# Nazukixv/LiteASR

Measured on AMD Instinct MI355X. Metric: utterances/sec (U2-Conformer+CTC, 80-d fbank T≈1000) at 1/2/4/8 MI355X, higher is better.
Workload: dtype bf16; 1 GPU; U2-Conformer-small hybrid CTC-attention training step (fwd+loss+bwd+allreduce+clip+Noam/Adam); model=U2 enc 12x conformer d256 H4 ff2048, dec 6x, V 4233, global_batch=32, per_gpu_batch=32, seq_len=1000, label_len=40, parallelism=dp1, launch=hipgraph, ranks_seen=1, rank_launcher=env

## Files before the change

### liteasr_amd/csrc/gemm.hip

```cpp
#include "gemm_kernel.h"
#include <algorithm>


template <bool AKC, bool BKC, typename TC>
void launch_bf16(const GemmP& p, int BM, int BN, int ks, int nw, bool glds, dim3 grid, hipStream_t st);
#define LASR_EXTERN_LAUNCH(ak, bk)                                                                         \
  extern template void launch_bf16<ak, bk, float>(const GemmP&, int, int, int, int, bool, dim3, hipStream_t); \
  extern template void launch_bf16<ak, bk, bf16_t>(const GemmP&, int, int, int, int, bool, dim3, hipStream_t);
LASR_EXTERN_LAUNCH(true, true)
LASR_EXTERN_LAUNCH(true, false)
LASR_EXTERN_LAUNCH(false, true)
LASR_EXTERN_LAUNCH(false, false)
#undef LASR_EXTERN_LAUNCH

template <typename TC>
static void dispatch(const GemmP& p, bool akc, bool bkc, int bf16in, int BM, int BN, int ks, int nw, bool glds,
                     dim3 grid, hipStream_t st) {
  if (bf16in) {
    if (akc && bkc) launch_bf16<true, true, TC>(p, BM, BN, ks, nw, glds, grid, st);
    else if (akc) launch_bf16<true, false, TC>(p, BM, BN, ks, nw, glds, grid, st);
    else if (bkc) launch_bf16<false, true, TC>(p, BM, BN, ks, nw, glds, grid, st);
    else launch_bf16<false, false, TC>(p, BM, BN, ks, nw, glds, grid, st);
  } else {
    if (akc && bkc) gemm_f32_kernel<true, true, TC><<<grid, 256, 0, st>>>(p);
// ... 191 lines not shown
  LASR_CHECK_ARG(grid.y <= 65535 && grid.z <= 65535, "lasr_gemm: grid too large");
  const bool rs_fused = a->rowsum && glds && !akc;
  if (rs_fused) {
    p.rowsum = a->rowsum;
    if (split > 1) p.rs_ws = p.ws + (int64_t)split * batch * a->M * a->N;
  }
  if (a->c_dtype == LASR_F32) dispatch<float>(p, akc, bkc, bf, BM, BN, ks, nw, glds, grid, st);
  else dispatch<bf16_t>(p, akc, bkc, bf, BM, BN, ks, nw, glds, grid, st);
  int rc = lasr_check_launch("lasr_gemm");
  if (!rc && split > 1 && a->split_k >= 0 && post) {
    const int r = post->launch(p, post->ctx, st);
    if (r < 0) return r;
    post->done = r;
    if (r) {
      rc = lasr_check_launch("lasr_gemm/splitk_reduce_post");
      if (rc || !a->rowsum || rs_fused) return rc;
    }
  }
  if (!rc && split > 1 && a->split_k >= 0 && !(post && post->done)) {
    const int64_t total = (int64_t)a->M * a->N * batch;
    const int nblk = (int)std::min<int64_t>(cdiv(p.v4 ? total / 4 : total, 256), 4096);
    if (a->c_dtype == LASR_F32) splitk_reduce_kernel<float><<<nblk, 256, 0, st>>>(p);
    else splitk_reduce_kernel<bf16_t><<<nblk, 256, 0, st>>>(p);
    rc = lasr_check_launch("lasr_gemm/splitk_reduce");
  }
  if (rc || !a->rowsum || rs_fused) return rc;
  const int64_t used = split > 1 ? (int64_t)split * batch * a->M * a->N : 0;
  LASR_CHECK_ARG(a->workspace && a->workspace_bytes / 4 > used, "lasr_gemm: no workspace left for the rowsum");
  return lasr_colsum(a->A, a->in_dtype, a->K, a->M, a->lda_k, a->rowsum, 1, (float*)a->workspace + used,
                     a->workspace_bytes / 4 - used, stream);
}


int launch_dw_group(const DwGroupP& g, int BM, int BN, int blocks, hipStream_t st);
static int dw_group_lpt = 1;
extern "C" int lasr_gemm_dw_group_order(int longest_first) {
  dw_group_lpt = longest_first != 0;
  return LASR_OK;
}

extern "C" int lasr_gemm_dw_group(const lasr_gemm_args* args, int n, void* stream) {
  LASR_CHECK_ARG(args && n >= 1 && n <= LASR_DW_GROUP_MAX, "lasr_gemm_dw_group: 1..%d problems", LASR_DW_GROUP_MAX);
  DwGroupP g = {};
  g.n = n;
  int ord[LASR_DW_GROUP_MAX];
  int64_t work[LASR_DW_GROUP_MAX];
  for (int i = 0; i < n; ++i) {
    const lasr_gemm_args* a = args + i;
    int bm, bn, sp, ks;
    gemm_plan(a, &bm, &bn, &sp, &ks);
    work[i] = a->split_k == 1 || sp <= 1 ? a->K : cdiv(a->K, sp);
    ord[i] = i;
  }
  if (dw_group_lpt)
    std::stable_sort(ord, ord + n, [&](int x, int y) { return work[x] > work[y]; });
  int BM0 = 0, BN0 = 0, blocks = 0;
  for (int i = 0; i < n; ++i) {
    const lasr_gemm_args* a = args + ord[i];
    LASR_CHECK_ARG(a->in_dtype == LASR_BF16 && a->c_dtype == LASR_F32, "lasr_gemm_dw_group: bf16 in, fp32 partials");
    LASR_CHECK_ARG(a->lda_m == 1 && a->lda_k != 1 && a->ldb_n == 1 && a->ldb_k != 1,
                   "lasr_gemm_dw_group: A M-contiguous and B N-contiguous (dW = dY^T X)");
    const bool direct = a->split_k == 1;
    LASR_CHECK_ARG((direct || (a->split_k < 0 && a->workspace)) && (a->batch <= 1) && a->M > 0 && a->N > 0 &&
                       a->K > 0,
                   "lasr_gemm_dw_group: partials-only problems with a workspace, or direct (split_k 1) ones");
    LASR_CHECK_ARG(!direct || (a->C && a->ldc >= a->N && (a->beta == 0.f || a->beta == 1.f) && a->alpha == 1.f &&
                               !a->alpha_dev),
                   "lasr_gemm_dw_group: a direct problem needs C, ldc >= N, beta 0 or 1, alpha 1");
    LASR_CHECK_ARG(i == 0 || direct == (g.direct[0] != 0), "lasr_gemm_dw_group: direct and split problems mixed");
    LASR_CHECK_ARG(!a->act && !a->zout && !a->aux && !a->res && a->drop_p <= 0.f && !a->bias,
                   "lasr_gemm_dw_group: no epilogue");
    LASR_CHECK_ARG(gemm_uses_glds(a), "lasr_gemm_dw_group: operands not LDS-DMA eligible");
    int BM, BN, split, ks;
    gemm_plan(a, &BM, &BN, &split, &ks);
    if (direct) split = 2;
    LASR_CHECK_ARG(split > 1, "lasr_gemm_dw_group: plan is not a split-K launch");
    if (((BM == 128 && BN == 64) || (BM == 64 && BN == 128)) && a->M >= 128 && a->N >= 128) {
      BM = BN = 128;
      if (a->M >= 256 && a->N >= 256 && !direct) {
        BM = 256;
        BN = 128;
      }
    }
    LASR_CHECK_ARG(i == 0 || (BM == BM0 && BN == BN0), "lasr_gemm_dw_group: problems plan different tiles");
    BM0 = BM;
    BN0 = BN;
    if (direct) split = 1;
    g.M[i] = a->M; g.N[i] = a->N; g.K[i] = a->K;
    g.split[i] = split;
    g.kchunk[i] = direct ? a->K : (int)(cdiv(cdiv(a->K, split), 32) * 32);
    g.direct[i] = direct;
    g.C[i] = (float*)a->C; g.ldc[i] = a->ldc; g.beta[i] = a->beta; g.rowsum[i] = a->rowsum;
    g.v4[i] = a->N % 4 == 0 && aligned16(direct ? a->C : a->workspace);
    g.A[i] = a->A; g.lda[i] = a->lda_k;
    g.B[i] = a->B; g.ldb[i] = a->ldb_k;
    g.ws[i] = (float*)a->workspace;
    g.rs_ws[i] = a->rowsum && !direct ? (float*)a->workspace + (int64_t)split * a->M * a->N : nullptr;
    g.start[i] = blocks;
    const int64_t nb = cdiv(a->M, BM) * cdiv(a->N, BN) * (int64_t)split;
    LASR_CHECK_ARG(blocks + nb + 8 < (1ll << 31), "lasr_gemm_dw_group: too many blocks");
    blocks += (int)cdiv(nb, 8) * 8;
  }
  g.start[n] = blocks;
  static const int slice_xcd = [] { const char* e = getenv("LASR_DW_SLICE_XCD"); return e && e[0] ? atoi(e) : 1; }();
  g.slice_xcd = slice_xcd;
  LASR_CHECK_ARG(launch_dw_group(g, BM0, BN0, blocks, (hipStream_t)stream) == 0,
                 "lasr_gemm_dw_group: no grouped instance for tile %dx%d", BM0, BN0);
  return lasr_check_launch("lasr_gemm_dw_group");
}
```

### liteasr_amd/csrc/gemm_group.hip

```cpp
#include "gemm_kernel.h"

int launch_dw_group(const DwGroupP& g, int BM, int BN, int blocks, hipStream_t st) {
  if (BM == 64 && BN == 64) gemm_dw_group_kernel<64, 64, 3, 3><<<blocks, 256, 0, st>>>(g);
  else if (BM == 64 && BN == 128) gemm_dw_group_kernel<64, 128, 3, 2><<<blocks, 256, 0, st>>>(g);
  else if (BM == 128 && BN == 64) gemm_dw_group_kernel<128, 64, 3, 2><<<blocks, 256, 0, st>>>(g);
  else if (BM == 128 && BN == 128) gemm_dw_group_kernel<128, 128, 2, 2><<<blocks, 256, 0, st>>>(g);
  else if (BM == 256 && BN == 128) gemm_dw_group_kernel<256, 128, 3, 1, 8><<<blocks, 512, 0, st>>>(g);
  else return -1;
  return 0;
}
```

### liteasr_amd/csrc/gemm_kernel.h

```cpp
#pragma once
#include "common.h"
#include "tile.h"

#include <cstring>
#include <type_traits>

#ifndef LASR_EXP
#define LASR_EXP 0
#endif


struct ConvG {
  int B, T1, F1, T2, F2, C;
  int M2;
  int cls;
  int q32, r32;
  const bf16_t* zero;
  const float* x;
  int T0, F0;
  float* w1part;
  int w1rb;
};
typedef ConvG ConvGeom;
enum { G_LIN = 0, G_FWD = 1, G_DW = 2, G_DX = 3 };
// ... 530 lines not shown
#pragma unroll
    for (int i = 0; i < FM; ++i) {
      const int m = mr + i * 16;
      if (m >= p.M) continue;
#pragma unroll
      for (int j = 0; j < FN; ++j) {
        const int n = nc + j * 16;
        if (n >= p.N) continue;
        float* dst = wsp + (int64_t)m * p.N + n;
        const float a[4] = {acc[i][j][0], acc[i][j][1], acc[i][j][2], acc[i][j][3]};
        if (p.v4 && n + 4 <= p.N) stv<4>(dst, a);
        else
          for (int q = 0; q < 4 && n + q < p.N; ++q) dst[q] = a[q];
      }
    }
    return;
  }
#pragma unroll
  for (int i = 0; i < FM; ++i) {
    const int m = mr + i * 16;
    if (m >= p.M) continue;
#pragma unroll
    for (int j = 0; j < FN; ++j) {
      const int n = nc + j * 16;
      if (n >= p.N) continue;
      const float a[4] = {acc[i][j][0], acc[i][j][1], acc[i][j][2], acc[i][j][3]};
      if (p.v4 && n + 4 <= p.N) epi_store4<TC, true>(p, dkey, z1, z2, z, m, n, 4, a, al);
      else epi_store4<TC, false>(p, dkey, z1, z2, z, m, n, min(4, p.N - n), a, al);
    }
  }
}

template <int BM, int BN, int NW>
LASR_DEV void dx_w1_epilogue(const GemmP& p, f32x4 (&acc)[BM / 32][BN / (8 * NW)], char* smem, int m0, int n0,
                             const int64_t* dxrow, const float (&xr)[(9 * BM + NW * 64 - 1) / (NW * 64)]) {
  static_assert(BN == 256 && NW == 4, "conv1 weight gradient: 4 columns per lane over a 256-column tile");
  constexpr int NT = NW * 64, WCOLS = NW / 2;
  constexpr int WM = BM / 2, WN = BN / WCOLS, FM = WM / 16, FN = WN / 16;
  constexpr int LDB = BN + 8;
  constexpr int RPW = BM / NW;
  constexpr int XN = (9 * BM + NT - 1) / NT;
  static_assert(BM * LDB * 2 + BM * 12 * 4 <= 73728 && NW * 10 * BN * 4 <= BM * LDB * 2, "LDS budget");
  bf16_t* tb = reinterpret_cast<bf16_t*>(smem);
  float* xs = reinterpret_cast<float*>(smem + BM * LDB * 2);
  const int tid = threadIdx.x, lane = tid & 63;
  const int wid = __builtin_amdgcn_readfirstlane(tid >> 6);
  const int wr = wid / WCOLS, wc = wid % WCOLS;
  const bf16_t* y1 = (const bf16_t*)p.aux;
  uint2 ya[RPW];
#pragma unroll
  for (int i = 0; i < RPW; ++i) {
    const int r = wid + NW * i;
    ya[i] = m0 + r < p.M ? *(const uint2*)(y1 + dxrow[r] + n0 + 4 * lane) : make_uint2(0u, 0u);
  }
  {
    const int rq = (lane >> 4) * 4, cl = lane & 15;
#pragma unroll
    for (int i = 0; i < FM; ++i)
#pragma unroll
      for (int j = 0; j < FN; ++j) {
        const int r = wr * WM + i * 16 + cl, c = wc * WN + j * 16 + rq;
        *(uint2*)(tb + r * LDB + c) = make_uint2(pk_bf16(acc[i][j][0], acc[i][j][1]), pk_bf16(acc[i][j][2], acc[i][j][3]));
      }
#pragma unroll
    for (int i = 0; i < XN; ++i) {
      const int e = i * NT + tid;
// ... 102 lines not shown
    for (int i = 0; i < PER; ++i) {
      const int P = i * NT + tid, k = P / CPR, ps = P % CPR;
      const int ls = ((((ps >> 1) ^ htr<R_TILE>(k))) << 1) | (ps & 1);
      const int gc = min(n0 + ls * 8, ((N + 7) & ~7) - 8);
      noff[i] = tbase + gc;
      const int m = kbeg + k;
      f2[i] = m % g.F2;
      const int t = m / g.F2;
      t2[i] = t % g.T2;
      b[i] = t / g.T2;
    }
  }
  LASR_DEV void issue(const ConvG& g, const bf16_t* base, bf16_t* dst, int tid) {
    const int wid = tid >> 6;
    const int last = ((g.B * g.T1 - g.T1 + 2 * (g.T2 - 1)) * g.F1 + 2 * (g.F2 - 1)) * g.C;
#pragma unroll
    for (int i = 0; i < PER; ++i) {
      const int rb = b[i] < g.B ? ((b[i] * g.T1 + 2 * t2[i]) * g.F1 + 2 * f2[i]) * g.C : last;
      __builtin_amdgcn_global_load_lds((gptr_t)(base + rb + noff[i]), (lptr_t)(dst + (i * NT + wid * 64) * 8),
                                       16, 0, 0);
      f2[i] += g.r32;
      t2[i] += g.q32;
      if (f2[i] >= g.F2) { f2[i] -= g.F2; t2[i] += 1; }
      while (t2[i] >= g.T2) { t2[i] -= g.T2; b[i] += 1; }
    }
  }
};

LASR_DEV int xcd_remap(int orig, int nwg) {
  const int xcd = orig & 7, q8 = nwg >> 3, r8 = nwg & 7;
  return (xcd < r8 ? xcd * (q8 + 1) : r8 * (q8 + 1) + (xcd - r8) * q8) + (orig >> 3);
}

template <int BM, int BN, bool AKC, bool BKC, typename TC, int S, int G, int KS, int NW = 4, int EPI = EPI_RT>
LASR_DEV void gemm_glds_tile(const GemmP& p, const int tx, const int ty, const int zz) {
  static_assert(G == G_LIN || (G == G_DW ? (!AKC && !BKC) : (AKC && (G == G_FWD) == BKC)),
                "gather instance operand orientation");
  static_assert(KS == 1 || KS == 2, "k sub-tiles per ring stage");
  static_assert(NW == 4 || NW == 8, "4 waves (2 x 2) or 8 waves (2 x 4)");
  constexpr int BK = 32;
  constexpr int NT = NW * 64, WCOLS = NW / 2;
  constexpr int WM = BM / 2, WN = BN / WCOLS, FM = WM / 16, FN = WN / 16;
  constexpr int TILE = (BM + BN) * BK;
  constexpr int STAGE = KS * TILE;
  constexpr int MAIN_BYTES = S * STAGE * 2;
  constexpr int EPI_BYTES = WM * (BN + 4) * 4;
  constexpr int GL = (BM + BN) * 4 / NT;
  __shared__ __attribute__((aligned(16))) char smem_epi[MAIN_BYTES > EPI_BYTES ? MAIN_BYTES : EPI_BYTES];
  bf16_t* smem = reinterpret_cast<bf16_t*>(smem_epi);
  const int tid = threadIdx.x, lane = tid & 63, wid = tid >> 6;
  const int wr = wid / WCOLS, wc = wid % WCOLS;

  const int s = zz % p.split_k, z = zz / p.split_k;
  const int z1 = z / p.batch_div, z2 = z % p.batch_div;
  const bf16_t* A = (const bf16_t*)p.A + z1 * p.sa1 + z2 * p.sa2;
  const bf16_t* B = (const bf16_t*)p.B + z1 * p.sb1 + z2 * p.sb2;
  const int m0 = ty * BM, n0 = tx * BN;
  const int kbeg = s * p.kchunk;
  const int kend = min(p.K, kbeg + p.kchunk);
  const int nk = kend > kbeg ? (kend - kbeg + BK - 1) / BK : 0;
  const int64_t lda = AKC ? p.lda_m : p.lda_k, ldb = BKC ? p.ldb_n : p.ldb_k;

  f32x4 acc[FM][FN];
#pragma unroll
  for (int i = 0; i < FM; ++i)
#pragma unroll
    for (int j = 0; j < FN; ++j) acc[i][j] = (f32x4){0.f, 0.f, 0.f, 0.f};

  const int nfull = (kend - kbeg) > 0 ? (kend - kbeg) / BK : 0;
  [[maybe_unused]] ConvRowsKC<BM, NT> ga;
  [[maybe_unused]] ConvRowsDW<BN, NT> gb;
  if constexpr (G == G_FWD) ga.init_fwd(p.cv, m0, p.M, tid);
  if constexpr (G == G_DX) ga.init_dx(p.cv, m0, p.M, tid);
  [[maybe_unused]] __shared__ int64_t dxrow[G == G_DX ? BM : 1];
  if constexpr (G == G_DX)
    for (int r = tid; r < BM; r += NT) dxrow[r] = dx_row(p.cv, min(m0 + r, p.M - 1));
  constexpr bool W1 = G == G_DX && EPI == EPI_AUX_RELU_W1;
  constexpr int XN = W1 ? (9 * BM + NT - 1) / NT : 1;
  [[maybe_unused]] float xr[XN];
  if constexpr (W1) {
    const ConvG& g = p.cv;
    const int pt = g.cls >> 1, pf = g.cls & 1;
    const int nI = (g.T1 - pt + 1) >> 1, nJ = (g.F1 - pf + 1) >> 1;
#pragma unroll
    for (int i = 0; i < XN; ++i) {
      const int e = i * NT + tid, r = e / 9, k = e - 9 * r;
      xr[i] = 0.f;
      if (e < 9 * BM) {
        const int m = min(m0 + r, p.M - 1);
        const int j = m % nJ, t = m / nJ, ii = t % nI, b = t / nI;
        const int kh = k / 3, kw = k - 3 * kh;
        xr[i] = g.x[((int64_t)b * g.T0 + 2 * (2 * ii + pt) + kh) * g.F0 + 2 * (2 * j + pf) + kw];
      }
    }
  }
  if constexpr (G == G_DW) gb.init(p.cv, n0, p.N, kbeg, tid);
  auto issue_sub = [&](const int k0, bf16_t* dst) {
    if (LASR_EXP & 4) return;
    if constexpr (G == G_LIN) {
      glds_tile<BM, AKC, NT>(A, lda, m0, p.M, k0, dst, tid);
      glds_tile<BN, BKC, NT>(B, ldb, n0, p.N, k0, dst + BM * BK, tid);
    } else if constexpr (G == G_FWD) {
// ... 36 lines not shown
    }
#pragma unroll
    for (int j = 0; j < FN; ++j) {
      if constexpr (BKC) bfr[j] = frag<BN, true>(cur + BM * BK, wc * WN + j * 16, lane);
      else frag_tr_raw_at(lds_addr(cur + BM * BK), boff[j], rb + 2 * j);
    }
    if constexpr (!AKC) {
      tie_lgkm<2 * FM>(ra);
#pragma unroll
      for (int i = 0; i < FM; ++i) af[i] = frag_from_raw(ra + 2 * i);
    }
    if constexpr (!BKC) {
      tie_lgkm<2 * FN>(rb);
#pragma unroll
      for (int j = 0; j < FN; ++j) bfr[j] = frag_from_raw(rb + 2 * j);
    }
    if (LASR_EXP & 1) {
#pragma unroll
      for (int i = 0; i < FM; ++i) acc[i][0][0] += (float)af[i][0] + (float)bfr[0][i & 1];
      return;
    }
#pragma unroll
    for (int i = 0; i < FM; ++i)
#pragma unroll
      for (int j = 0; j < FN; ++j)
        acc[i][j] = __builtin_amdgcn_mfma_f32_16x16x32_bf16(bfr[j], af[i], acc[i][j], 0, 0, 0);
  };

  const bool do_rs = !AKC && p.rowsum != nullptr && tx == 0;
  float rs[8];
#pragma unroll
  for (int q = 0; q < 8; ++q) rs[q] = 0.f;

  const int nst = nfull / KS;
#pragma unroll
  for (int t = 0; t < S - 1; ++t)
    if (t < nst) issue(t);

  for (int kt = 0; kt < nst; ++kt) {
    const int after = min(S - 2, nst - 1 - kt);
    wait_ring<S, GL * KS>(after);
    lds_barrier();
    if (kt + S - 1 < nst) issue(kt + S - 1);
#pragma unroll
    for (int u = 0; u < KS; ++u) compute(smem + (kt % S) * STAGE + u * TILE);
    if constexpr (!AKC)
      if (do_rs)
#pragma unroll
        for (int u = 0; u < KS; ++u) rowsum_tile<BM, NT>(smem + (kt % S) * STAGE + u * TILE, tid, rs);
  }
  if constexpr (KS > 1) {
    for (int j = nst * KS; j < nfull; ++j) {
      __syncthreads();
      issue_sub(kbeg + j * BK, smem);
      wait_vmcnt<0>();
      lds_barrier();
      compute(smem);
      if constexpr (!AKC)
        if (do_rs) rowsum_tile<BM, NT>(smem, tid, rs);
    }
  }
  if (G == G_LIN && nfull < nk) {
    __syncthreads();
    TileLoader<BM, AKC, NT> la;
    TileLoader<BN, BKC, NT> lb;
    const int k0 = kbeg + nfull * BK;
    la.load(A, AKC ? p.lda_m : 0, AKC ? 0 : p.lda_k, m0, p.M, k0, kend, true, tid);
    lb.load(B, BKC ? p.ldb_n : 0, BKC ? 0 : p.ldb_k, n0, p.N, k0, kend, true, tid);
    la.store(smem, tid);
    lb.store(smem + BM * BK, tid);
    __syncthreads();
    compute(smem);
    if constexpr (!AKC)
      if (do_rs) rowsum_tile<BM, NT>(smem, tid, rs);
  }
  __syncthreads();
  if constexpr (!AKC) {
    if (do_rs) {
      constexpr int CH = BM / 8, KG = NT / CH;
      float* red = reinterpret_cast<float*>(smem_epi);
      const int c = tid % CH, kg = tid / CH;
#pragma unroll
      for (int q = 0; q < 8; ++q) red[kg * BM + 8 * c + q] = rs[q];
      __syncthreads();
      if (tid < BM) {
        float t = 0.f;
        for (int g = 0; g < KG; ++g) t += red[g * BM + tid];
        const int m = m0 + tid;
        if (m < p.M) {
          if (p.split_k > 1) p.rs_ws[(int64_t)s * p.M + m] = t;
          else p.rowsum[m] += t;
        }
      }
      __syncthreads();
    }
  }
  if constexpr (W1) {
    dx_w1_epilogue<BM, BN, NW>(p, acc, smem_epi, m0, n0, dxrow, xr);
    return;
  }
  if (p.split_k > 1) gemm_epilogue_direct<BM, BN, TC, NW>(p, acc, m0, n0, s, z, z1, z2);
  else gemm_epilogue<BM, BN, TC, true, G, NW, EPI>(p, acc, smem_epi, m0, n0, s, z, z1, z2, dxrow);
}

LASR_DEV void dw_tile_order(int wg, int nx, int ny, bool n_major, int& tx, int& ty) {
  if (n_major) { tx = wg / ny; ty = wg % ny; }
  else { tx = wg % nx; ty = wg / nx; }
}

template <int BM, int BN, bool AKC, bool BKC, typename TC, int S, int MINB = 3, int G = G_LIN, int KS = 1,
          int NW = 4, int EPI = EPI_RT>
__global__ __launch_bounds__(NW * 64, MINB * NW / 4) void gemm_bf16_glds_kernel(GemmP p) {
  const int nx = gridDim.x, ny = gridDim.y;
  const int wg = xcd_remap(blockIdx.y * nx + blockIdx.x, nx * ny);
  int tx, ty;
  dw_tile_order(wg, nx, ny, !AKC && !BKC && G == G_LIN && p.N > p.M, tx, ty);
  gemm_glds_tile<BM, BN, AKC, BKC, TC, S, G, KS, NW, EPI>(p, tx, ty, blockIdx.z);
}

#define LASR_DW_GROUP_MAX 8
struct DwGroupP {
  int n;
  int start[LASR_DW_GROUP_MAX + 1];
  int M[LASR_DW_GROUP_MAX], N[LASR_DW_GROUP_MAX], K[LASR_DW_GROUP_MAX];
  int split[LASR_DW_GROUP_MAX], kchunk[LASR_DW_GROUP_MAX], v4[LASR_DW_GROUP_MAX];
  const void* A[LASR_DW_GROUP_MAX];
  const void* B[LASR_DW_GROUP_MAX];
  int64_t lda[LASR_DW_GROUP_MAX], ldb[LASR_DW_GROUP_MAX];
  float* ws[LASR_DW_GROUP_MAX];
  float* rs_ws[LASR_DW_GROUP_MAX];
  int slice_xcd;
  int direct[LASR_DW_GROUP_MAX];
  float* C[LASR_DW_GROUP_MAX];
  int64_t ldc[LASR_DW_GROUP_MAX];
  float beta[LASR_DW_GROUP_MAX];
  float* rowsum[LASR_DW_GROUP_MAX];
};

template <int BM, int BN, int S, int MINB, int NW = 4>
__global__ __launch_bounds__(NW * 64, MINB * NW / 4) void gemm_dw_group_kernel(DwGroupP g) {
  const int blk = blockIdx.x;
  int i = 0;
  for (int j = 1; j < g.n; ++j)
    if (blk >= g.start[j]) i = j;
  const int ntx = (g.N[i] + BN - 1) / BN, nty = (g.M[i] + BM - 1) / BM, ntile = ntx * nty;
  const int local = blk - g.start[i];
  if (local >= ntile * g.split[i]) return;
  GemmP p = {};
  p.M = g.M[i]; p.N = g.N[i]; p.K = g.K[i]; p.batch = 1; p.batch_div = 1;
  p.A = g.A[i]; p.lda_m = 1; p.lda_k = g.lda[i];
  p.B = g.B[i]; p.ldb_n = 1; p.ldb_k = g.ldb[i];
  p.split_k = g.split[i]; p.kchunk = g.kchunk[i]; p.ws = g.ws[i]; p.v4 = g.v4[i];
  p.rowsum = g.rs_ws[i];
  p.rs_ws = g.rs_ws[i];
  p.alpha = 1.f;
  if (g.direct[i]) {
    p.C = g.C[i]; p.ldc = g.ldc[i]; p.beta = g.beta[i];
    p.rowsum = g.rowsum[i]; p.rs_ws = nullptr; p.ws = nullptr;
    p.c_vec = ((uintptr_t)p.C & 15) == 0 && p.ldc % 8 == 0;
    p.epi_mode = p.c_vec && p.beta == 0.f ? 0 : 2;
  }
  int tile, slice;
  const int sp = g.split[i], per = 8 / (sp > 0 ? sp : 1);
  if (g.slice_xcd && 8 % sp == 0 && ntile % per == 0 && (ntile * sp) % 8 == 0) {
    const int x = local & 7, q = local >> 3, run = ntile / per;
    slice = x / per;
    tile = (x % per) * run + q;
  } else {
    tile = xcd_remap(local % ntile, ntile);
    slice = local / ntile;
  }
  int tx, ty;
  dw_tile_order(tile, ntx, nty, p.N > p.M, tx, ty);
  gemm_glds_tile<BM, BN, false, false, float, S, G_LIN, 2, NW>(p, tx, ty, slice);
}

template <bool AKC, bool BKC, typename TC>
__global__ __launch_bounds__(256) void gemm_f32_kernel(GemmP p) {
  constexpr int BM = 64, BN = 64, BK = 16, LD = BK + 1;
  __shared__ float As[BM * LD], Bs[BN * LD];
  const int tid = threadIdx.x, lane = tid & 63, wid = tid >> 6;
  const int wr = wid >> 1, wc = wid & 1;
  const int zz = blockIdx.z;
  const int s = zz % p.split_k, z = zz / p.split_k;
  const int z1 = z / p.batch_div, z2 = z % p.batch_div;
  const float* A = (const float*)p.A + z1 * p.sa1 + z2 * p.sa2;
  const float* B = (const float*)p.B + z1 * p.sb1 + z2 * p.sb2;
  const int m0 = blockIdx.y * BM, n0 = blockIdx.x * BN;
  const int kbeg = s * p.kchunk;
  const int kend = min(p.K, kbeg + p.kchunk);

  f32x4 acc[2][2];
#pragma unroll
// ... 136 lines not shown
```

### liteasr_amd/kernels.py

```python

from __future__ import annotations

import contextlib
import os
import ctypes as C
import math
from types import SimpleNamespace
from typing import Optional

import torch

from . import _native as N

_DT = {torch.float32: N.F32, torch.bfloat16: N.BF16}


def dt(t: torch.Tensor) -> int:
    try:
        return _DT[t.dtype]
    except KeyError:
        raise TypeError(f"unsupported dtype {t.dtype}") from None


def ptr(t: Optional[torch.Tensor]):
# ... 5 lines not shown


class _Workspace:

    def __init__(self):
        self.buf = {}
        self.frozen = False

    def get(self, nfloats: int, device) -> torch.Tensor:
        nfloats = max(int(nfloats), 1)
        key = torch.device(device).index
        b = self.buf.get(key)
        if b is None or b.numel() < nfloats:
            if self.frozen or torch.cuda.is_current_stream_capturing():
                raise RuntimeError(
                    "workspace growth during graph capture; run a warm-up step first"
                )
            b = torch.empty(int(nfloats * 1.25) + 1024, dtype=torch.float32, device=device)
            self.buf[key] = b
        return b


WS = _Workspace()


class _Deferred:

    def __init__(self):
        self.depth = 0
        self.segs = []
        self.gemms = []
        self.held = []
        self.done = []


_DEFER = _Deferred()


@contextlib.contextmanager
def deferred_reductions(hold=False, on_done=None):
    if _DEFER.depth and (hold or on_done is not None):
        raise RuntimeError("deferred_reductions: hold / on_done inside another deferred block would be dropped")
    _DEFER.depth += 1
    ok = False
    try:
        yield
        ok = True
    finally:
        _DEFER.depth -= 1
        if _DEFER.depth == 0:
            if hold and ok:
                if _DEFER.gemms:
                    _flush_gemm_group()
                _DEFER.held.extend(_DEFER.segs)
                _DEFER.segs = []
                if on_done is not None:
                    _DEFER.done.append(on_done)
            else:
                if on_done is not None:
                    _DEFER.done.append(on_done)
                flush_reductions()


def held_reductions():
    return len(_DEFER.held)


def _defer(part, P, Ncols, out0, out1=None, split=None, accumulate=True):
    _DEFER.segs.append((part, int(P), int(Ncols), out0, out1, int(split if split is not None else Ncols),
                        int(accumulate)))


DW_GROUP = True
_GROUP_TILES = {(64, 64): (64, 64), (64, 128): (128, 128), (128, 64): (128, 128)}
DW_GROUP_SPLIT_DIV = {(64, 64): 4, (128, 128): 2}
DW_DIRECT_MIN_TILES = 0


SMALL_GRID_SPLIT = True
SMALL_GRID_TILES = 128


def _group_div(key):
    d = DW_GROUP_SPLIT_DIV
    return d.get(key, 1) if isinstance(d, dict) else d
_GROUP_MAX = 8


DW_GROUP_LPT = True
_dw_order_set = [None]


def _flush_gemm_group():
    q, _DEFER.gemms = _DEFER.gemms, []
    if _dw_order_set[0] != DW_GROUP_LPT:
        N.call("lasr_gemm_dw_group_order", int(DW_GROUP_LPT))
        _dw_order_set[0] = DW_GROUP_LPT
    byt = {}
    for key, args, refs in q:
        byt.setdefault(key, []).append(args)
    for key, lst in byt.items():
        for i in range(0, len(lst), _GROUP_MAX):
            chunk = lst[i:i + _GROUP_MAX]
            arr = (N.GemmArgs * len(chunk))(*chunk)
            N.call("lasr_gemm_dw_group", arr, len(chunk), stream())


def _flush_node_end(segs):
    if _DEFER.gemms:
        _flush_gemm_group()
    if segs:
        arr = (N.ReduceSeg * len(segs))()
        for i, (part, P, Ncols, o0, o1, split, acc) in enumerate(segs):
            arr[i] = N.ReduceSeg(ptr(part), Ncols, P, acc, ptr(o0), ptr(o1), split)
        N.call("lasr_reduce_multi", arr, len(segs), stream())


def flush_reductions():
    segs = _DEFER.held + _DEFER.segs
    _DEFER.held, _DEFER.segs = [], []
    done, _DEFER.done = _DEFER.done, []
    if segs or _DEFER.gemms:
        _flush_node_end(segs)
    for fn in done:
        fn()



GEMM_NARROW_TILES = True
_narrow_set = [None]


def _split(t: torch.Tensor):
    nb = t.dim() - 2
    assert 0 <= nb <= 2, "gemm operands take at most 2 batch dims"
    st = t.stride()
    sh = t.shape
    if nb == 0:
        return (0, 0), (1, 1), st[0], st[1]
    if nb == 1:
        return (st[0], 0), (sh[0], 1), st[1], st[2]
    return (st[0], st[1]), (sh[0], sh[1]), st[2], st[3]


def gemm(
    a: torch.Tensor,
    b: torch.Tensor,
    c: torch.Tensor,
    *,
    alpha: float = 1.0,
    alpha_dev: Optional[torch.Tensor] = None,
# ... 70 lines not shown
        assert z1 * z2 == 1 and a_m == 1, "rowsum needs batch 1 and an M-contiguous A"
        args.rowsum = ptr(rowsum)
    if split_k != 1 or rowsum is not None:
        ns = 64 if split_k <= 0 else split_k
        need = ns * z1 * z2 * M * Nn + (ns + 128) * M if rowsum is not None else ns * z1 * z2 * M * Nn
        ws = WS.get(need, c.device)
        args.workspace, args.workspace_bytes = ptr(ws), ws.numel() * 4
    if plan_only:
        tm, tn, sp, fl = C.c_int(), C.c_int(), C.c_int(), C.c_int()
        N.call("lasr_gemm_plan", C.byref(args), C.byref(tm), C.byref(tn), C.byref(sp), C.byref(fl))
        if plan_only == "flags":
            return tm.value, tn.value, sp.value, fl.value
        return tm.value, tn.value, sp.value
    if (_DEFER.depth and split_k == 0 and not auto_split and beta in (0.0, 1.0) and alpha == 1.0 and alpha_dev is None
            and bias is None and act == N.ACT_NONE and zout is None and aux is None and res is None
            and drop_p <= 0.0 and z1 * z2 == 1 and c.dtype == torch.float32 and c.is_contiguous()):
        tm, tn, sp, fl = C.c_int(), C.c_int(), C.c_int(), C.c_int()
        N.call("lasr_gemm_plan", C.byref(args), C.byref(tm), C.byref(tn), C.byref(sp), C.byref(fl))
        sp = sp.value
        grouped = (group and DW_GROUP and (tm.value, tn.value) in _GROUP_TILES
                   and (fl.value & 1) and a_m == 1 and b_n == 1 and a.dtype == torch.bfloat16)
        if (grouped and DW_DIRECT_MIN_TILES > 0 and _GROUP_TILES[(tm.value, tn.value)] == (128, 128)
                and ((M + 127) // 128) * ((Nn + 127) // 128) >= DW_DIRECT_MIN_TILES):
            args.split_k = 1
            args.workspace, args.workspace_bytes = None, 0
            _DEFER.gemms.append(((128, 128, "direct"), N.GemmArgs.from_buffer_copy(args), (a, b, c, rowsum)))
            return c
        div = _group_div(_GROUP_TILES[(tm.value, tn.value)]) if grouped else 1
        if grouped and (div > 1 or sp < 2):
            sp = max(2, sp // max(1, div))
            args.split_k = -sp
            N.call("lasr_gemm_plan", C.byref(args), C.byref(tm), C.byref(tn), C.byref(C.c_int()), C.byref(fl))
            grouped = (tm.value, tn.value) in _GROUP_TILES and bool(fl.value & 1)
        if sp > 1:
            nrs = (sp + 128) * M if rowsum is not None else 0
            part = torch.empty(sp * M * Nn + nrs, dtype=torch.float32, device=c.device)
            args.split_k = -sp
            args.workspace, args.workspace_bytes = ptr(part), part.numel() * 4
            if grouped:
                key = _GROUP_TILES[(tm.value, tn.value)]
                _DEFER.gemms.append((key, N.GemmArgs.from_buffer_copy(args), (a, b)))
            else:
                N.call("lasr_gemm", C.byref(args), stream())
            _defer(part, sp, M * Nn, c, accumulate=beta == 1.0)
            if rowsum is not None and fl.value & 2:
                _defer(part[sp * M * Nn:], sp, M, rowsum)
            return c
    if ln_fwd is not None:
        g_, b_, eps, y, mean, rstd = ln_fwd
        assert c.dtype == torch.float32 and c.is_contiguous() and z1 * z2 == 1 and rowsum is None
        N.call("lasr_gemm_ln_fwd", C.byref(args), ptr(g_), ptr(b_), float(eps), ptr(y), dt(y), ptr(mean), ptr(rstd),
               stream())
        return c
    if qbias is not None:
        dqu, dqv, B_, T_, H_, dk_, dqkv, du, dv = qbias
        assert c.dtype == dqu.dtype == dqv.dtype == dqkv.dtype
        D_ = H_ * dk_
        nchunk = (B_ * T_ + 63) // 64
        part = torch.empty(nchunk * 2 * D_, dtype=torch.float32, device=c.device)
        N.call("lasr_gemm_qbias_bwd", C.byref(args), ptr(dqu), ptr(dqv), dt(dqu), B_, T_, H_, dk_, ptr(dqkv),
               dqkv.stride(0), ptr(part), part.numel(), stream())
        if _DEFER.depth:
            _defer(part, nchunk, 2 * D_, du, dv, split=D_)
        else:
            arr = (N.ReduceSeg * 1)()
            arr[0] = N.ReduceSeg(ptr(part), 2 * D_, nchunk, 1, ptr(du), ptr(dv), D_)
# ... 719 lines not shown
```

Measured before the change: 3386 utterances/sec.

## Hold weight-gradient GEMMs across layers and run split-K slices serially in-block

```diff
diff --git a/liteasr_amd/csrc/gemm.hip b/liteasr_amd/csrc/gemm.hip
--- a/liteasr_amd/csrc/gemm.hip
+++ b/liteasr_amd/csrc/gemm.hip
@@ -247,7 +247,7 @@
 }
 
 
-int launch_dw_group(const DwGroupP& g, int BM, int BN, int blocks, hipStream_t st);
+int launch_dw_group(const DwGroupP& g, int BM, int BN, int blocks, bool serial, hipStream_t st);
 static int dw_group_lpt = 1;
 extern "C" int lasr_gemm_dw_group_order(int longest_first) {
   dw_group_lpt = longest_first != 0;
@@ -260,18 +260,28 @@
   g.n = n;
   int ord[LASR_DW_GROUP_MAX];
   int64_t work[LASR_DW_GROUP_MAX];
+  auto planned = [](const lasr_gemm_args* a) {
+    lasr_gemm_args b = *a;
+    if (b.split_k <= -2 && !b.workspace) {
+      b.workspace = (void*)(uintptr_t)16;
+      b.workspace_bytes = INT64_MAX;
+    }
+    return b;
+  };
   for (int i = 0; i < n; ++i) {
-    const lasr_gemm_args* a = args + i;
+    const lasr_gemm_args pa = planned(args + i), *a = &pa;
     int bm, bn, sp, ks;
     gemm_plan(a, &bm, &bn, &sp, &ks);
     work[i] = a->split_k == 1 || sp <= 1 ? a->K : cdiv(a->K, sp);
     ord[i] = i;
   }
-  if (dw_group_lpt)
+  if (dw_group_lpt && !(args[0].split_k <= -2 && !args[0].workspace))
     std::stable_sort(ord, ord + n, [&](int x, int y) { return work[x] > work[y]; });
   int BM0 = 0, BN0 = 0, blocks = 0;
+  bool all_serial = false;
   for (int i = 0; i < n; ++i) {
-    const lasr_gemm_args* a = args + ord[i];
+    const bool serial = args[ord[i]].split_k <= -2 && !args[ord[i]].workspace;
+    const lasr_gemm_args pa = planned(args + ord[i]), *a = &pa;
     LASR_CHECK_ARG(a->in_dtype == LASR_BF16 && a->c_dtype == LASR_F32, "lasr_gemm_dw_group: bf16 in, fp32 partials");
     LASR_CHECK_ARG(a->lda_m == 1 && a->lda_k != 1 && a->ldb_n == 1 && a->ldb_k != 1,
                    "lasr_gemm_dw_group: A M-contiguous and B N-contiguous (dW = dY^T X)");
@@ -279,6 +289,11 @@
     LASR_CHECK_ARG((direct || (a->split_k < 0 && a->workspace)) && (a->batch <= 1) && a->M > 0 && a->N > 0 &&
                        a->K > 0,
                    "lasr_gemm_dw_group: partials-only problems with a workspace, or direct (split_k 1) ones");
+    LASR_CHECK_ARG(!serial || (a->C && a->ldc >= a->N && (a->beta == 0.f || a->beta == 1.f) && a->alpha == 1.f &&
+                               !a->alpha_dev && a->split_k >= -64),
+                   "lasr_gemm_dw_group: a serial problem needs C, ldc >= N, beta 0 or 1, alpha 1, <= 64 slices");
+    LASR_CHECK_ARG(i == 0 || serial == all_serial, "lasr_gemm_dw_group: serial and slab problems mixed");
+    all_serial = serial;
     LASR_CHECK_ARG(!direct || (a->C && a->ldc >= a->N && (a->beta == 0.f || a->beta == 1.f) && a->alpha == 1.f &&
                                !a->alpha_dev),
                    "lasr_gemm_dw_group: a direct problem needs C, ldc >= N, beta 0 or 1, alpha 1");
@@ -306,20 +321,21 @@
     g.kchunk[i] = direct ? a->K : (int)(cdiv(cdiv(a->K, split), 32) * 32);
     g.direct[i] = direct;
     g.C[i] = (float*)a->C; g.ldc[i] = a->ldc; g.beta[i] = a->beta; g.rowsum[i] = a->rowsum;
-    g.v4[i] = a->N % 4 == 0 && aligned16(direct ? a->C : a->workspace);
+    g.v4[i] = serial ? a->N % 4 == 0 && aligned16(a->C) && a->ldc % 4 == 0
+                     : a->N % 4 == 0 && aligned16(direct ? a->C : a->workspace);
     g.A[i] = a->A; g.lda[i] = a->lda_k;
     g.B[i] = a->B; g.ldb[i] = a->ldb_k;
-    g.ws[i] = (float*)a->workspace;
-    g.rs_ws[i] = a->rowsum && !direct ? (float*)a->workspace + (int64_t)split * a->M * a->N : nullptr;
+    g.ws[i] = serial ? nullptr : (float*)a->workspace;
+    g.rs_ws[i] = a->rowsum && !direct && !serial ? (float*)a->workspace + (int64_t)split * a->M * a->N : nullptr;
     g.start[i] = blocks;
-    const int64_t nb = cdiv(a->M, BM) * cdiv(a->N, BN) * (int64_t)split;
+    const int64_t nb = cdiv(a->M, BM) * cdiv(a->N, BN) * (int64_t)(serial ? 1 : split);
     LASR_CHECK_ARG(blocks + nb + 8 < (1ll << 31), "lasr_gemm_dw_group: too many blocks");
     blocks += (int)cdiv(nb, 8) * 8;
   }
   g.start[n] = blocks;
   static const int slice_xcd = [] { const char* e = getenv("LASR_DW_SLICE_XCD"); return e && e[0] ? atoi(e) : 1; }();
   g.slice_xcd = slice_xcd;
-  LASR_CHECK_ARG(launch_dw_group(g, BM0, BN0, blocks, (hipStream_t)stream) == 0,
+  LASR_CHECK_ARG(launch_dw_group(g, BM0, BN0, blocks, all_serial, (hipStream_t)stream) == 0,
                  "lasr_gemm_dw_group: no grouped instance for tile %dx%d", BM0, BN0);
   return lasr_check_launch("lasr_gemm_dw_group");
 }
diff --git a/liteasr_amd/csrc/gemm_group.hip b/liteasr_amd/csrc/gemm_group.hip
--- a/liteasr_amd/csrc/gemm_group.hip
+++ b/liteasr_amd/csrc/gemm_group.hip
@@ -1,6 +1,14 @@
 #include "gemm_kernel.h"
 
-int launch_dw_group(const DwGroupP& g, int BM, int BN, int blocks, hipStream_t st) {
+static_assert(sizeof(DwGroupP) <= 4096, "DwGroupP must fit the kernel-argument block");
+
+int launch_dw_group(const DwGroupP& g, int BM, int BN, int blocks, bool serial, hipStream_t st) {
+  if (serial) {
+    if (BM == 64 && BN == 64) gemm_dw_group_kernel<64, 64, 3, 3, 4, true><<<blocks, 256, 0, st>>>(g);
+    else if (BM == 256 && BN == 128) gemm_dw_group_kernel<256, 128, 3, 1, 8, true><<<blocks, 512, 0, st>>>(g);
+    else return -1;
+    return 0;
+  }
   if (BM == 64 && BN == 64) gemm_dw_group_kernel<64, 64, 3, 3><<<blocks, 256, 0, st>>>(g);
   else if (BM == 64 && BN == 128) gemm_dw_group_kernel<64, 128, 3, 2><<<blocks, 256, 0, st>>>(g);
   else if (BM == 128 && BN == 64) gemm_dw_group_kernel<128, 64, 3, 2><<<blocks, 256, 0, st>>>(g);
diff --git a/liteasr_amd/csrc/gemm_kernel.h b/liteasr_amd/csrc/gemm_kernel.h
--- a/liteasr_amd/csrc/gemm_kernel.h
+++ b/liteasr_amd/csrc/gemm_kernel.h
@@ -586,6 +586,40 @@
 }
 
 template <int BM, int BN, int NW>
+LASR_DEV void gemm_epilogue_serial(const GemmP& p, f32x4 (&tot)[BM / 32][BN / (8 * NW)], int m0, int n0) {
+  constexpr int WCOLS = NW / 2;
+  constexpr int WM = BM / 2, WN = BN / WCOLS, FM = WM / 16, FN = WN / 16;
+  const int lane = threadIdx.x & 63, wid = threadIdx.x >> 6;
+  const int wr = wid / WCOLS, wc = wid % WCOLS;
+  const int mr = m0 + wr * WM + (lane & 15), nc = n0 + wc * WN + 4 * (lane >> 4);
+  const bool accum = p.beta != 0.f;
+  float* C = (float*)p.C;
+#pragma unroll
+  for (int i = 0; i < FM; ++i) {
+    const int m = mr + i * 16;
+    if (m >= p.M) continue;
+#pragma unroll
+    for (int j = 0; j < FN; ++j) {
+      const int n = nc + j * 16;
+      if (n >= p.N) continue;
+      float* dst = C + (int64_t)m * p.ldc + n;
+      float a[4] = {tot[i][j][0], tot[i][j][1], tot[i][j][2], tot[i][j][3]};
+      if (p.v4 && n + 4 <= p.N) {
+        if (accum) {
+          float c[4];
+          ldv<4>(dst, c);
+#pragma unroll
+          for (int q = 0; q < 4; ++q) a[q] = c[q] + a[q];
+        }
+        stv<4>(dst, a);
+      } else {
+        for (int q = 0; q < 4 && n + q < p.N; ++q) dst[q] = accum ? dst[q] + a[q] : a[q];
+      }
+    }
+  }
+}
+
+template <int BM, int BN, int NW>
 LASR_DEV void dx_w1_epilogue(const GemmP& p, f32x4 (&acc)[BM / 32][BN / (8 * NW)], char* smem, int m0, int n0,
                              const int64_t* dxrow, const float (&xr)[(9 * BM + NW * 64 - 1) / (NW * 64)]) {
   static_assert(BN == 256 && NW == 4, "conv1 weight gradient: 4 columns per lane over a 256-column tile");
@@ -754,10 +788,13 @@
   return (xcd < r8 ? xcd * (q8 + 1) : r8 * (q8 + 1) + (xcd - r8) * q8) + (orig >> 3);
 }
 
-template <int BM, int BN, bool AKC, bool BKC, typename TC, int S, int G, int KS, int NW = 4, int EPI = EPI_RT>
+template <int BM, int BN, bool AKC, bool BKC, typename TC, int S, int G, int KS, int NW = 4, int EPI = EPI_RT,
+          bool SERIAL = false>
 LASR_DEV void gemm_glds_tile(const GemmP& p, const int tx, const int ty, const int zz) {
   static_assert(G == G_LIN || (G == G_DW ? (!AKC && !BKC) : (AKC && (G == G_FWD) == BKC)),
                 "gather instance operand orientation");
+  static_assert(!SERIAL || (G == G_LIN && !AKC && !BKC && std::is_same<TC, float>::value && EPI == EPI_RT),
+                "serial slices: fp32 weight gradients only");
   static_assert(KS == 1 || KS == 2, "k sub-tiles per ring stage");
   static_assert(NW == 4 || NW == 8, "4 waves (2 x 2) or 8 waves (2 x 4)");
   constexpr int BK = 32;
@@ -773,14 +810,15 @@
   const int tid = threadIdx.x, lane = tid & 63, wid = tid >> 6;
   const int wr = wid / WCOLS, wc = wid % WCOLS;
 
-  const int s = zz % p.split_k, z = zz / p.split_k;
+  int s = SERIAL ? 0 : zz % p.split_k;
+  const int z = SERIAL ? 0 : zz / p.split_k;
   const int z1 = z / p.batch_div, z2 = z % p.batch_div;
   const bf16_t* A = (const bf16_t*)p.A + z1 * p.sa1 + z2 * p.sa2;
   const bf16_t* B = (const bf16_t*)p.B + z1 * p.sb1 + z2 * p.sb2;
   const int m0 = ty * BM, n0 = tx * BN;
-  const int kbeg = s * p.kchunk;
-  const int kend = min(p.K, kbeg + p.kchunk);
-  const int nk = kend > kbeg ? (kend - kbeg + BK - 1) / BK : 0;
+  int kbeg = s * p.kchunk;
+  int kend = min(p.K, kbeg + p.kchunk);
+  int nk = kend > kbeg ? (kend - kbeg + BK - 1) / BK : 0;
   const int64_t lda = AKC ? p.lda_m : p.lda_k, ldb = BKC ? p.ldb_n : p.ldb_k;
 
   f32x4 acc[FM][FN];
@@ -789,7 +827,7 @@
 #pragma unroll
     for (int j = 0; j < FN; ++j) acc[i][j] = (f32x4){0.f, 0.f, 0.f, 0.f};
 
-  const int nfull = (kend - kbeg) > 0 ? (kend - kbeg) / BK : 0;
+  int nfull = (kend - kbeg) > 0 ? (kend - kbeg) / BK : 0;
   [[maybe_unused]] ConvRowsKC<BM, NT> ga;
   [[maybe_unused]] ConvRowsDW<BN, NT> gb;
   if constexpr (G == G_FWD) ga.init_fwd(p.cv, m0, p.M, tid);
@@ -892,68 +930,103 @@
 #pragma unroll
   for (int q = 0; q < 8; ++q) rs[q] = 0.f;
 
-  const int nst = nfull / KS;
-#pragma unroll
-  for (int t = 0; t < S - 1; ++t)
-    if (t < nst) issue(t);
-
-  for (int kt = 0; kt < nst; ++kt) {
-    const int after = min(S - 2, nst - 1 - kt);
-    wait_ring<S, GL * KS>(after);
-    lds_barrier();
-    if (kt + S - 1 < nst) issue(kt + S - 1);
-#pragma unroll
-    for (int u = 0; u < KS; ++u) compute(smem + (kt % S) * STAGE + u * TILE);
-    if constexpr (!AKC)
-      if (do_rs)
-#pragma unroll
-        for (int u = 0; u < KS; ++u) rowsum_tile<BM, NT>(smem + (kt % S) * STAGE + u * TILE, tid, rs);
-  }
-  if constexpr (KS > 1) {
-    for (int j = nst * KS; j < nfull; ++j) {
+  [[maybe_unused]] f32x4 tot[SERIAL ? FM : 1][SERIAL ? FN : 1];
+  [[maybe_unused]] float rs_tot = 0.f;
+  if constexpr (SERIAL)
+#pragma unroll
+    for (int i = 0; i < FM; ++i)
+#pragma unroll
+      for (int j = 0; j < FN; ++j) tot[i][j] = (f32x4){0.f, 0.f, 0.f, 0.f};
+  [[maybe_unused]] int sl = 0;
+  do {
+    if constexpr (SERIAL) {
+      s = sl;
+      kbeg = s * p.kchunk;
+      kend = min(p.K, kbeg + p.kchunk);
+      nk = kend > kbeg ? (kend - kbeg + BK - 1) / BK : 0;
+      nfull = (kend - kbeg) > 0 ? (kend - kbeg) / BK : 0;
+#pragma unroll
+      for (int i = 0; i < FM; ++i)
+#pragma unroll
+        for (int j = 0; j < FN; ++j) acc[i][j] = (f32x4){0.f, 0.f, 0.f, 0.f};
+#pragma unroll
+      for (int q = 0; q < 8; ++q) rs[q] = 0.f;
+    }
+    const int nst = nfull / KS;
+#pragma unroll
+    for (int t = 0; t < S - 1; ++t)
+      if (t < nst) issue(t);
+
+    for (int kt = 0; kt < nst; ++kt) {
+      const int after = min(S - 2, nst - 1 - kt);
+      wait_ring<S, GL * KS>(after);
+      lds_barrier();
+      if (kt + S - 1 < nst) issue(kt + S - 1);
+#pragma unroll
+      for (int u = 0; u < KS; ++u) compute(smem + (kt % S) * STAGE + u * TILE);
+      if constexpr (!AKC)
+        if (do_rs)
+#pragma unroll
+          for (int u = 0; u < KS; ++u) rowsum_tile<BM, NT>(smem + (kt % S) * STAGE + u * TILE, tid, rs);
+    }
+    if constexpr (KS > 1) {
+      for (int j = nst * KS; j < nfull; ++j) {
+        __syncthreads();
+        issue_sub(kbeg + j * BK, smem);
+        wait_vmcnt<0>();
+        lds_barrier();
+        compute(smem);
+        if constexpr (!AKC)
+          if (do_rs) rowsum_tile<BM, NT>(smem, tid, rs);
+      }
+    }
+    if (G == G_LIN && nfull < nk) {
       __syncthreads();
-      issue_sub(kbeg + j * BK, smem);
-      wait_vmcnt<0>();
-      lds_barrier();
+      TileLoader<BM, AKC, NT> la;
+      TileLoader<BN, BKC, NT> lb;
+      const int k0 = kbeg + nfull * BK;
+      la.load(A, AKC ? p.lda_m : 0, AKC ? 0 : p.lda_k, m0, p.M, k0, kend, true, tid);
+      lb.load(B, BKC ? p.ldb_n : 0, BKC ? 0 : p.ldb_k, n0, p.N, k0, kend, true, tid);
+      la.store(smem, tid);
+      lb.store(smem + BM * BK, tid);
+      __syncthreads();
       compute(smem);
       if constexpr (!AKC)
         if (do_rs) rowsum_tile<BM, NT>(smem, tid, rs);
     }
-  }
-  if (G == G_LIN && nfull < nk) {
     __syncthreads();
-    TileLoader<BM, AKC, NT> la;
-    TileLoader<BN, BKC, NT> lb;
-    const int k0 = kbeg + nfull * BK;
-    la.load(A, AKC ? p.lda_m : 0, AKC ? 0 : p.lda_k, m0, p.M, k0, kend, true, tid);
-    lb.load(B, BKC ? p.ldb_n : 0, BKC ? 0 : p.ldb_k, n0, p.N, k0, kend, true, tid);
-    la.store(smem, tid);
-    lb.store(smem + BM * BK, tid);
-    __syncthreads();
-    compute(smem);
-    if constexpr (!AKC)
-      if (do_rs) rowsum_tile<BM, NT>(smem, tid, rs);
-  }
-  __syncthreads();
-  if constexpr (!AKC) {
-    if (do_rs) {
-      constexpr int CH = BM / 8, KG = NT / CH;
-      float* red = reinterpret_cast<float*>(smem_epi);
-      const int c = tid % CH, kg = tid / CH;
-#pragma unroll
-      for (int q = 0; q < 8; ++q) red[kg * BM + 8 * c + q] = rs[q];
-      __syncthreads();
-      if (tid < BM) {
-        float t = 0.f;
-        for (int g = 0; g < KG; ++g) t += red[g * BM + tid];
-        const int m = m0 + tid;
-        if (m < p.M) {
-          if (p.split_k > 1) p.rs_ws[(int64_t)s * p.M + m] = t;
-          else p.rowsum[m] += t;
+    if constexpr (!AKC) {
+      if (do_rs) {
+        constexpr int CH = BM / 8, KG = NT / CH;
+        float* red = reinterpret_cast<float*>(smem_epi);
+        const int c = tid % CH, kg = tid / CH;
+#pragma unroll
+        for (int q = 0; q < 8; ++q) red[kg * BM + 8 * c + q] = rs[q];
+        __syncthreads();
+        if (tid < BM) {
+          float t = 0.f;
+          for (int g = 0; g < KG; ++g) t += red[g * BM + tid];
+          const int m = m0 + tid;
+          if constexpr (SERIAL) {
+            rs_tot += t;
+          } else if (m < p.M) {
+            if (p.split_k > 1) p.rs_ws[(int64_t)s * p.M + m] = t;
+            else p.rowsum[m] += t;
+          }
         }
-      }
-      __syncthreads();
-    }
+        __syncthreads();
+      }
+    }
+    if constexpr (SERIAL)
+#pragma unroll
+      for (int i = 0; i < FM; ++i)
+#pragma unroll
+        for (int j = 0; j < FN; ++j) tot[i][j] += acc[i][j];
+  } while (SERIAL && ++sl < p.split_k);
+  if constexpr (SERIAL) {
+    if (do_rs && tid < BM && m0 + tid < p.M) p.rowsum[m0 + tid] += rs_tot;
+    gemm_epilogue_serial<BM, BN, NW>(p, tot, m0, n0);
+    return;
   }
   if constexpr (W1) {
     dx_w1_epilogue<BM, BN, NW>(p, acc, smem_epi, m0, n0, dxrow, xr);
@@ -978,7 +1051,7 @@
   gemm_glds_tile<BM, BN, AKC, BKC, TC, S, G, KS, NW, EPI>(p, tx, ty, blockIdx.z);
 }
 
-#define LASR_DW_GROUP_MAX 8
+#define LASR_DW_GROUP_MAX 32
 struct DwGroupP {
   int n;
   int start[LASR_DW_GROUP_MAX + 1];
@@ -997,7 +1070,7 @@
   float* rowsum[LASR_DW_GROUP_MAX];
 };
 
-template <int BM, int BN, int S, int MINB, int NW = 4>
+template <int BM, int BN, int S, int MINB, int NW = 4, bool SERIAL = false>
 __global__ __launch_bounds__(NW * 64, MINB * NW / 4) void gemm_dw_group_kernel(DwGroupP g) {
   const int blk = blockIdx.x;
   int i = 0;
@@ -1005,7 +1078,7 @@
     if (blk >= g.start[j]) i = j;
   const int ntx = (g.N[i] + BN - 1) / BN, nty = (g.M[i] + BM - 1) / BM, ntile = ntx * nty;
   const int local = blk - g.start[i];
-  if (local >= ntile * g.split[i]) return;
+  if (local >= (SERIAL ? ntile : ntile * g.split[i])) return;
   GemmP p = {};
   p.M = g.M[i]; p.N = g.N[i]; p.K = g.K[i]; p.batch = 1; p.batch_div = 1;
   p.A = g.A[i]; p.lda_m = 1; p.lda_k = g.lda[i];
@@ -1019,6 +1092,14 @@
     p.rowsum = g.rowsum[i]; p.rs_ws = nullptr; p.ws = nullptr;
     p.c_vec = ((uintptr_t)p.C & 15) == 0 && p.ldc % 8 == 0;
     p.epi_mode = p.c_vec && p.beta == 0.f ? 0 : 2;
+  }
+  if constexpr (SERIAL) {
+    p.C = g.C[i]; p.ldc = g.ldc[i]; p.beta = g.beta[i];
+    p.rowsum = g.rowsum[i]; p.rs_ws = nullptr; p.ws = nullptr;
+    int tx, ty;
+    dw_tile_order(xcd_remap(local, ntile), ntx, nty, p.N > p.M, tx, ty);
+    gemm_glds_tile<BM, BN, false, false, float, S, G_LIN, 2, NW, EPI_RT, true>(p, tx, ty, 0);
+    return;
   }
   int tile, slice;
   const int sp = g.split[i], per = 8 / (sp > 0 ? sp : 1);
diff --git a/liteasr_amd/kernels.py b/liteasr_amd/kernels.py
--- a/liteasr_amd/kernels.py
+++ b/liteasr_amd/kernels.py
@@ -61,6 +61,9 @@
         self.gemms = []
         self.held = []
         self.done = []
+        self.holding = False
+        self.held_gemms = []
+        self.held_layers = 0
 
 
 _DEFER = _Deferred()
@@ -70,6 +73,8 @@
 def deferred_reductions(hold=False, on_done=None):
     if _DEFER.depth and (hold or on_done is not None):
         raise RuntimeError("deferred_reductions: hold / on_done inside another deferred block would be dropped")
+    if _DEFER.depth == 0:
+        _DEFER.holding = bool(hold)
     _DEFER.depth += 1
     ok = False
     try:
@@ -78,6 +83,9 @@
     finally:
         _DEFER.depth -= 1
         if _DEFER.depth == 0:
+            _DEFER.holding = False
+            waiting = [q for q in _DEFER.gemms if _waits(q)]
+            _DEFER.gemms = [q for q in _DEFER.gemms if not _waits(q)]
             if hold and ok:
                 if _DEFER.gemms:
                     _flush_gemm_group()
@@ -85,14 +93,21 @@
                 _DEFER.segs = []
                 if on_done is not None:
                     _DEFER.done.append(on_done)
+                if waiting:
+                    _DEFER.held_gemms.extend(waiting)
+                    _DEFER.held_layers += 1
+                    if DW_HOLD_LAYERS and _DEFER.held_layers >= DW_HOLD_LAYERS:
+                        _flush_held_gemms()
             else:
+                if ok:
+                    _DEFER.held_gemms.extend(waiting)
                 if on_done is not None:
                     _DEFER.done.append(on_done)
                 flush_reductions()
 
 
 def held_reductions():
-    return len(_DEFER.held)
+    return len(_DEFER.held) + len(_DEFER.held_gemms)
 
 
 def _defer(part, P, Ncols, out0, out1=None, split=None, accumulate=True):
@@ -113,18 +128,64 @@
 def _group_div(key):
     d = DW_GROUP_SPLIT_DIV
     return d.get(key, 1) if isinstance(d, dict) else d
-_GROUP_MAX = 8
+_GROUP_MAX = 32
+
+DW_HOLD_GEMMS = True
+DW_SERIAL_MIN_TILES = 256
+DW_HOLD_LAYERS = 4
+
+
+def _waits(q):
+    return q[1].split_k <= -2 and not q[1].workspace
+
+
+def _serial_tiles(key, M, Nn):
+    if key == (64, 64):
+        return -(-M // 64) * -(-Nn // 64)
+    if M >= 256 and Nn >= 256:
+        return -(-M // 256) * -(-Nn // 128)
+    return -(-M // 128) * -(-Nn // 128)
+
+
+def _flush_held_gemms():
+    q, _DEFER.held_gemms = _DEFER.held_gemms, []
+    _DEFER.held_layers = 0
+    _set_dw_order()
+    byt = {}
+    for key, args, refs in q:
+        byt.setdefault(key, []).append((args, refs))
+    for key, lst in byt.items():
+        chunks = [lst[i:i + _GROUP_MAX] for i in range(0, len(lst), _GROUP_MAX)]
+        tiles = [sum(_serial_tiles(key, a.M, a.N) for a, _ in ch) for ch in chunks]
+        serial = (sum(tiles) >= DW_SERIAL_MIN_TILES and all(t >= DW_SERIAL_MIN_TILES for t in tiles[:-1])
+                  and (key == (64, 64) or all(a.M >= 256 and a.N >= 256 for a, _ in lst)))
+        if not serial:
+            for args, (a, b, c, rowsum) in lst:
+                sp, M, Nn = -args.split_k, args.M, args.N
+                nrs = (sp + 128) * M if rowsum is not None else 0
+                part = torch.empty(sp * M * Nn + nrs, dtype=torch.float32, device=c.device)
+                args.workspace, args.workspace_bytes = ptr(part), part.numel() * 4
+                _DEFER.held.append((part, sp, M * Nn, c, None, M * Nn, int(args.beta == 1.0)))
+                if rowsum is not None:
+                    _DEFER.held.append((part[sp * M * Nn:], sp, M, rowsum, None, M, 1))
+        for ch in chunks:
+            arr = (N.GemmArgs * len(ch))(*[a for a, _ in ch])
+            N.call("lasr_gemm_dw_group", arr, len(ch), stream())
 
 
 DW_GROUP_LPT = True
 _dw_order_set = [None]
 
 
-def _flush_gemm_group():
-    q, _DEFER.gemms = _DEFER.gemms, []
+def _set_dw_order():
     if _dw_order_set[0] != DW_GROUP_LPT:
         N.call("lasr_gemm_dw_group_order", int(DW_GROUP_LPT))
         _dw_order_set[0] = DW_GROUP_LPT
+
+
+def _flush_gemm_group():
+    q, _DEFER.gemms = _DEFER.gemms, []
+    _set_dw_order()
     byt = {}
     for key, args, refs in q:
         byt.setdefault(key, []).append(args)
@@ -146,6 +207,8 @@
 
 
 def flush_reductions():
+    if _DEFER.held_gemms:
+        _flush_held_gemms()
     segs = _DEFER.held + _DEFER.segs
     _DEFER.held, _DEFER.segs = [], []
     done, _DEFER.done = _DEFER.done, []
@@ -282,6 +345,13 @@
             args.split_k = -sp
             N.call("lasr_gemm_plan", C.byref(args), C.byref(tm), C.byref(tn), C.byref(C.c_int()), C.byref(fl))
             grouped = (tm.value, tn.value) in _GROUP_TILES and bool(fl.value & 1)
+        if (sp > 1 and grouped and (_DEFER.holding or _DEFER.held_gemms) and DW_HOLD_GEMMS and sp <= 64
+                and (M * Nn) % 4 == 0 and (rowsum is None or (M % 4 == 0 and fl.value & 2))):
+            args.split_k = -sp
+            args.workspace, args.workspace_bytes = None, 0
+            key = _GROUP_TILES[(tm.value, tn.value)]
+            _DEFER.gemms.append((key, N.GemmArgs.from_buffer_copy(args), (a, b, c, rowsum)))
+            return c
         if sp > 1:
             nrs = (sp + 128) * M if rowsum is not None else 0
             part = torch.empty(sp * M * Nn + nrs, dtype=torch.float32, device=c.device)
```

Result: faster. 3489 utterances/sec (median of 6 runs) (+3.0%).
